# European-XFEL/xFrame

Hardware: AMD Instinct MI355X
Metric: MTIP iterations/sec, 128 q-shells x L_max=32 (higher is better)
Workload: dtype f64 (complex128); 1 GPU; BASELINE config 4: 128 shells x L_max=32, grid 128x64x128, 8 restarts per GPU on 3 streams, tutorial schedule (HIO/SW/ER, ft_stab on), fused step; restarts_per_gpu=8, restarts_total=8, streams_per_gpu=3, engines_take_turns=True, parallelism=restart-sharded x1, step_mode=fused

## Files before the change

### xframe_amd/csrc/k_sht.hip

```cpp
#include "mtip_internal.h"
#include "k_sht_common.h"
#include <cmath>
#include <cstdlib>

void build_legendre_tables(mtip_ctx* c, const double* cos_theta) {
    const int L = c->L, nt = c->nt;
    std::vector<int> poff(L + 2);
    for (int m = 0; m <= L + 1; ++m) poff[m] = m * (L + 1) - m * (m - 1) / 2;
    const size_t rows = (size_t)(L + 1) * (L + 2) / 2;
    std::vector<double> P(rows * nt);
    std::vector<double2> AB(rows, make_double2(0.0, 0.0));
    const double pi = 3.14159265358979323846;
    for (int t = 0; t < nt; ++t) {
        const double x = cos_theta[t];
        const double s = std::sqrt(std::fmax(0.0, 1.0 - x * x));
        double pmm = std::sqrt(1.0 / (4.0 * pi));
        for (int m = 0; m <= L; ++m) {
            if (m > 0) pmm = -std::sqrt((2.0 * m + 1.0) / (2.0 * m)) * s * pmm;
            P[(size_t)(poff[m]) * nt + t] = pmm;
            if (m < L) {
                double p2 = pmm;
                double p1 = std::sqrt(2.0 * m + 3.0) * x * pmm;
                P[(size_t)(poff[m] + 1) * nt + t] = p1;
                for (int l = m + 2; l <= L; ++l) {
                    const double a = std::sqrt((4.0 * l * l - 1.0) / ((double)l * l - (double)m * m));
                    const double b = std::sqrt((((double)l - 1.0) * (l - 1.0) - (double)m * m) / (4.0 * (l - 1.0) * (l - 1.0) - 1.0));
                    const double p = a * (x * p1 - b * p2);
                    P[(size_t)(poff[m] + l - m) * nt + t] = p;
                    AB[(size_t)poff[m] + l - m] = make_double2(a, b);
                    p2 = p1;
                    p1 = p;
                }
            }
        }
    }
    (void)mtip_copy(c, c->d_P, P.data(), P.size() * sizeof(double), hipMemcpyHostToDevice);
    (void)mtip_copy(c, c->d_poff, poff.data(), poff.size() * sizeof(int), hipMemcpyHostToDevice);
    if (c->d_AB != nullptr) (void)mtip_copy(c, c->d_AB, AB.data(), AB.size() * sizeof(double2), hipMemcpyHostToDevice);
    if (c->d_PT != nullptr) {
        const int nth = nt / 2;
        std::vector<double> PT((size_t)nth * rows);
        std::vector<int> lmtab(rows);
        for (int m = 0; m <= L; ++m)
            for (int l = m; l <= L; ++l) {
                const size_t idx = (size_t)poff[m] + l - m;
                lmtab[idx] = l | (m << 8);
                for (int t = 0; t < nth; ++t) PT[(size_t)t * rows + idx] = P[idx * nt + t];
            }
        (void)mtip_copy(c, c->d_PT, PT.data(), PT.size() * sizeof(double), hipMemcpyHostToDevice);
        (void)mtip_copy(c, c->d_lmtab, lmtab.data(), lmtab.size() * sizeof(int), hipMemcpyHostToDevice);
        c->chain_chunks = 0;
        if (c->d_PTc != nullptr) {
            std::vector<int> lmc(3 * 256, -1);
            std::vector<double> PTc((size_t)nth * 3 * 256, 0.0);
            int t = 0;
            bool fits = true;
            for (int m = 0; m <= L && fits; ++m)
                for (int par = 0; par < 2 && fits; ++par)
                    for (int l0 = m + par; l0 <= L; l0 += 6) {
                        if (t >= 256) { fits = false; break; }
                        for (int u = 0; u < 3; ++u) {
                            const int l = l0 + 2 * u;
// ... 191 lines not shown
            if (slot != nullptr) {
                const long long rows_per_b = (long long)Nq * nt;
                oo += (long long)slot[(row / rows_per_b) * SL_N + which] * B * rows_per_b * np;
            }
            if (EPI == EPI_MODULUS) {
                const double2 Fv = Fin[o];
                const double I = cabs2(Fv);
                const bool ok = (I >= 0.0) && (v.x >= 0.0);
                const double mult = ok ? sqrt(v.x / I) : 0.0;
                v = cscale(Fv, mult);
            } else if (EPI == EPI_SCALE_SHELL) {
                v = cscale(v, shell_scale[q]);
            }
            grid[oo] = v;
        }
    }
}

static void fft_launch_dims(const mtip_ctx* c, long long nrows, dim3* grid, dim3* block, size_t* smem) {
    const int T = c->np / 2;
    int R = 256 / T;
    if (R < 1) R = 1;
    *block = dim3((unsigned)(R * T));
    *grid = dim3((unsigned)div_up(nrows, R));
    *smem = (size_t)2 * R * c->np * sizeof(double2);
}

static constexpr size_t SHT_LDS_MAX = 160 * 1024, SHT_WIDE_LDS_MAX = 158 * 1024;

static size_t wide_lds(const mtip_ctx* c, int r1, int r2, int nsplit, int* rp) {
    if (c->nt % (2 * nsplit) != 0) return 0;
    const int ntl = c->nt / nsplit;
    if (nsplit > 1 && (ntl / 2) % 32 != 0) return 0;
    const size_t fixed = (nsplit > 1 ? 0 : (size_t)c->np) + (size_t)ntl * c->nm + c->npairs;
    auto bytes = [&](int v) { return (fixed + std::max((size_t)c->nlm, (size_t)v * r1 * (r2 + 1))) * sizeof(double2); };
    *rp = largest_even_divisor_le(ntl, std::min(SW_THREADS / r2, SW_THREADS / r1));
    while (*rp >= 2 && bytes(*rp) > SHT_WIDE_LDS_MAX) *rp = largest_even_divisor_le(ntl, *rp - 2);
    return *rp >= 2 ? bytes(*rp) : 0;
}

static void plan_chain(const mtip_ctx* c, int r1, int r2, ShtPlan& p) {
    if (c->np > 128) return;
    const int TP = c->nt / 2;
    for (int gsz = 64; gsz <= SW_THREADS; gsz *= 2) {
        const int maxi = div_up(c->npairs, gsz);
        if (TP % (SW_THREADS / gsz) != 0 || maxi > 3) continue;
        p.chain_gsz = gsz;
        p.chain_thg = TP / (SW_THREADS / gsz);
        const bool reg_tab = c->np == 128 && p.chain_thg == 16 && maxi >= 2;
        p.chain_maxi = reg_tab ? maxi : (maxi == 1 ? 1 : 3);
        p.chain = !reg_tab ? SHT_CHAIN_RT
                : (p.chain_maxi == 3 && c->L == 32 && c->nt == 64 && c->chain_chunks > 0) ? SHT_CHAIN_L32 : SHT_CHAIN_REGTAB;
        break;
    }
    if (p.chain == SHT_CHAIN_OFF) return;
    const size_t tb = (size_t)(SW_THREADS / 64) * (64 / r2) * r1 * (r2 + 1);
    const size_t fixed = (size_t)c->np + (size_t)c->nt * c->nm + c->npairs;
    p.chain_lds = (fixed + std::max(std::max((size_t)c->nlm, tb), (size_t)SW_THREADS * p.chain_maxi * 2)) * sizeof(double2);
    if (p.chain_lds > SHT_WIDE_LDS_MAX) p.chain = SHT_CHAIN_OFF;
}

void plan_sht(mtip_ctx* c) {
    int cap = 5;
    if (const char* e = std::getenv("MTIP_SHT_TIER")) cap = std::min(std::max(std::atoi(e), 0), 5);
    ShtPlan p;
    const int nt = c->nt, np = c->np;
    const size_t z = sizeof(double2);
    int r1 = 0, r2 = 0;
    if (cap >= 2 && nt % 2 == 0 && reg_radices(np, &r1, &r2)) {
        p.fwd_rp = largest_even_divisor_le(nt, std::min(2 * SR_THREADS / r2, SR_THREADS / r1));
        p.inv_rp = largest_even_divisor_le(nt, std::min(SR_THREADS / r2, SR_THREADS / r1));
        p.fwd_lds = ((size_t)np + (size_t)p.fwd_rp * r1 * (r2 + 1)) * z;
        p.inv_lds = ((size_t)np + c->nlm + (size_t)p.inv_rp * c->nm + (size_t)p.inv_rp * r1 * (r2 + 1)) * z;
        if (p.fwd_rp >= 2 && p.inv_rp >= 2 && p.fwd_lds <= SHT_LDS_MAX && p.inv_lds <= SHT_LDS_MAX) {
            p.fwd = SHT_FWD_REG;
            p.inv = SHT_INV_REG;
        }
    }
    if (p.fwd == SHT_FWD_REG) {
        const int per = div_up(c->npairs, SR_THREADS);
        p.fwd_maxi = per <= 3 ? 3 : per <= 5 ? 5 : 9;
        const int th = p.fwd_rp / 4;
        if (cap >= 3 && p.fwd_rp % 4 == 0 && (th == 2 || th == 4 || th == 8) && (nt / 2) % th == 0 && per <= 5) {
            p.fwd = SHT_FWD_PAIR;
            p.fwd_th = th;
            p.fwd_lds = ((size_t)np + (size_t)(p.fwd_rp / 2) * r1 * (r2 + 1)) * z;
        }
        for (int ns = 1; cap >= 3 && ns <= 2 && p.inv != SHT_INV_WIDE; ++ns) {
            int rp = 0;
            const size_t lds = wide_lds(c, r1, r2, ns, &rp);
            if (lds == 0) continue;
// ... 103 lines not shown
```

### xframe_amd/csrc/k_sht_chain.hip

```cpp
#include "mtip_internal.h"
#include "k_sht_common.h"
#include "k_sht_legendre.h"

#define CHAIN_STAMP(i)                           \
    if constexpr (DBG) stamp[i] = clock64();
#define CHAIN_SEG(i)                             \
    if constexpr (DBG) {                         \
        const long long n_ = clock64();          \
        stamp[i] += n_ - tprev;                  \
        tprev = n_;                              \
    }

struct ChainArgs {
    const double2* coeff;
    double2* grid;
    const double* P;
    const double2* AB;
    const double* cost;
    const double2* twN_g;
    const double2* Fin;
    const int* slot;
    const uint16_t* mk;
    RealEpi re;
    int npairs, nt, L, Nq, which, B;
    double2* coeff_out;
    const double* PT;
    const int* lmtab;
    const double* PTc;
    const int* lmc;
    const double* gw;
    double norm;
    long long* dbg;
    int gsz, thg;
};

template <int EPI, int PRE, int R1, int R2, int MAXI, int THG, bool DBG, int LC, bool CHK>
__global__ void __launch_bounds__(SW_THREADS) k_sht_chain(ChainArgs a) {
    constexpr int N = R1 * R2;
    constexpr int AS = R2 + 1;
    constexpr int GSR = R1 * AS;
    HIP_DYNAMIC_SHARED(double2, sm)
    long long stamp[DBG ? MTIP_CHAIN_DBG_SLOTS : 1];
    long long tprev = 0;
    if constexpr (DBG) {
#pragma unroll
        for (int i = 0; i < MTIP_CHAIN_DBG_SLOTS; ++i) stamp[i] = 0;
    }
    const int L = LC > 0 ? LC : a.L, nt = a.nt, npairs = LC > 0 ? (LC + 1) * (LC + 2) / 2 : a.npairs, Nq = a.Nq, B = a.B;
    const int nm = 2 * L + 1;
    const int nlm = (L + 1) * (L + 1);
    double2* twN = sm;
    double2* Gs = sm + N;
    double2* ABs = Gs + (size_t)nt * nm;
    double2* cl = ABs + npairs;
    double2* Bm = cl;
    const int tid = threadIdx.x;
    const long long shell = blockIdx.x;
    const int q = (int)(shell % Nq);
    const double2* csrc = a.coeff + (size_t)shell * nlm;
    const int wave = __builtin_amdgcn_readfirstlane(tid >> 6), nw = blockDim.x >> 6;
    CHAIN_STAMP(0)
    LegendreStart ls;
    legendre_prefetch_first(ls, a.P, nt, L, nt >> 1, 0, wave, tid & 63);
    for (int e = tid; e < N; e += blockDim.x) sm[e] = a.twN_g[e];
    for (int e = tid; e < npairs; e += blockDim.x) ABs[e] = a.AB[e];
    for (int e = tid; e < nlm; e += blockDim.x) cl[e] = csrc[e];
    long long dst_shell = shell;
    if (a.slot != nullptr && a.which >= 0) dst_shell += (long long)a.slot[(shell / Nq) * SL_N + a.which] * B * Nq;
    double2* gdst = a.grid + (size_t)dst_shell * nt * N;
    const double2* fsrc = a.Fin ? a.Fin + (size_t)shell * nt * N : nullptr;
    const double2* rprev = nullptr;
    const uint16_t* rmk = nullptr;
    double err_num = 0.0, err_den = 0.0;
    if (EPI == EPI_REAL_UPDATE) {
        const int bb = (int)(shell / Nq);
        const int* sl = a.slot + bb * SL_N;
        const size_t gsh = (size_t)nt * N;
        rprev = a.re.prev + ((size_t)sl[SL_CUR] * B * Nq + shell) * gsh;
        gdst = a.re.out + ((size_t)sl[SL_OUT] * B * Nq + shell) * gsh;
        rmk = a.mk + ((size_t)sl[SL_SUP] * B * Nq + shell) * nt * R2;
    }
    const int gsz = a.gsz;
    const int thg = THG > 0 ? THG : a.thg;
    const int grp = __builtin_amdgcn_readfirstlane(tid / gsz);
    const int tg = tid - grp * gsz;
    constexpr bool SPLIT = R2 == 16;
    constexpr int RW = 64 / R2;
    constexpr int S1 = RW * R1;
    static_assert(S1 * (SPLIT ? 2 : 1) <= 64, "lane roles");
    const int lane = tid & 63;
    const int n_grp = (nt + RW - 1) / RW;
    double2* Bw = Bm + (size_t)wave * (RW * R1 * AS);
    const int r2l = lane / R2, n2 = lane - r2l * R2;
    const int hf = SPLIT ? lane / S1 : 0;
    const int t1 = lane - hf * S1;
    const bool role1 = SPLIT || lane < S1;
    const int r1l = (t1 / R1) % RW, k1 = t1 % R1;
    constexpr bool HAS_PRE = EPI == EPI_MODULUS || EPI == EPI_REAL_UPDATE;
    double2 pre[HAS_PRE ? R1 : 1];
    unsigned pre_m = 0;
    double pre_w = 0.0;
    auto load_pre = [&](int g) {
        const int rr = g * RW + r2l;
        if (HAS_PRE && g < n_grp && rr < nt) {
            const int th = rr >> 1;
            const int row = (rr & 1) ? (nt - 1 - th) : th;
#pragma unroll
            for (int n1 = 0; n1 < R1; ++n1) {
                const size_t o = (size_t)row * N + R2 * n1 + n2;
                if (EPI == EPI_MODULUS) pre[n1] = fsrc[o];
                if (EPI == EPI_REAL_UPDATE) pre[n1] = rprev[o];
            }
            if (EPI == EPI_REAL_UPDATE) {
                pre_m = rmk[row * R2 + n2];
                pre_w = a.re.wt[row];
            }
        }
    };
    int my_lm[MAXI];
#pragma unroll
    for (int u = 0; u < MAXI; ++u) my_lm[u] = CHK ? a.lmc[u * 256 + tg] : a.lmtab[min(tg + u * gsz, npairs - 1)];
    __syncthreads();
    CHAIN_STAMP(1)
    load_pre(wave);
    const RealFlags rflags = real_flags(a.re.rp, a.re.method);
    const bool add_prev = EPI == EPI_REAL_UPDATE && a.re.add_prev && q > 0 && (a.re.add_mask == nullptr || a.re.add_mask[shell / Nq] != 0);
    const double wr_q = EPI == EPI_REAL_UPDATE ? a.re.wr[q] : 0.0;
    legendre_synthesis_rows(ls, Gs, cl, ABs, a.P, a.cost, nt, L, nt >> 1, 0, wave, nw, tid & 63);
    CHAIN_STAMP(2)
    __syncthreads();
    CHAIN_STAMP(3)
    if constexpr (DBG) tprev = stamp[3];
    for (int g = wave; g < n_grp; g += nw) {
        {
            const int rr = g * RW + r1l;
            if (role1 && rr < nt) {
                const double2* gr = Gs + (size_t)rr * nm + L;
                double2 uv[R2];
#pragma unroll
                for (int k2 = 0; k2 < R2; ++k2) {
                    const int k = k1 + R1 * k2;
                    const bool lo = k <= L, hi = k >= N - L;
                    const double2 v = gr[lo ? k : (hi ? k - N : 0)];
                    uv[k2] = (lo || hi) ? v : make_double2(0.0, 0.0);
                }
                double2* br = Bw + (size_t)(r1l * R1 + k1) * AS;
                if constexpr (SPLIT) {
                    double2 yv[R2 / 2];
                    half_fft<R2, true>(uv, hf, yv);
#pragma unroll
                    for (int j = 0; j < R2 / 2; ++j) {
                        const int m2 = 2 * j + hf;
                        double2 w = twN[m2 * k1];
                        w.y = -w.y;
                        br[m2] = cmul(yv[j], w);
                    }
                } else {
                    SmallFFT<R2, true>::run(uv);
#pragma unroll
                    for (int m2 = 0; m2 < R2; ++m2) {
                        double2 w = twN[m2 * k1];
// ... 14 lines not shown
            const double2* br = Bw + (size_t)r2l * R1 * AS + n2;
#pragma unroll
            for (int q1 = 0; q1 < R1; ++q1) vv[q1] = br[q1 * AS];
            SmallFFT<R1, true>::run(vv);
            const int th = rr2 >> 1;
            const int row = (rr2 & 1) ? (nt - 1 - th) : th;
#pragma unroll
            for (int n1 = 0; n1 < R1; ++n1) {
                double2 v = vv[n1];
                const size_t o = (size_t)row * N + R2 * n1 + n2;
                if (EPI == EPI_MODULUS) {
                    const double2 Fv = pre[n1];
                    const double I = cabs2(Fv);
                    const bool ok = (I >= 0.0) && (v.x >= 0.0);
                    const double mult = ok ? sqrt(v.x / I) : 0.0;
                    v = cscale(Fv, mult);
                } else if (EPI == EPI_REAL_UPDATE) {
                    const double2 pv = pre[n1];
                    const double2 w = add_prev ? cadd(v, pv) : v;
                    double2 Pj;
                    v = real_update_point_flat(a.re.rp, rflags, a.re.beta, w, pv, ((pre_m >> n1) & 1u) != 0, Pj);
                    if (!a.re.err_use_mask || ((pre_m >> (8 + n1)) & 1u)) {
                        const double wg = wr_q * pre_w;
                        const double dx = w.x - Pj.x, dy = w.y - Pj.y;
                        err_num = fma(wg, dx * dx + dy * dy, err_num);
                        err_den = fma(wg, w.x * w.x + w.y * w.y, err_den);
                    }
                }
                gdst[o] = v;
                if (PRE == MTIP_PRE_SQUARE) v = make_double2(cabs2(v), 0.0);
                vv[n1] = v;
            }
        }
        load_pre(g + nw);
#pragma unroll
        for (int n1 = 0; n1 < R1; ++n1) {
            const double px = __shfl_xor(vv[n1].x, R2, 64), py = __shfl_xor(vv[n1].y, R2, 64);
            vv[n1] = (r2l & 1) ? make_double2(px - vv[n1].x, py - vv[n1].y)
                               : make_double2(vv[n1].x + px, vv[n1].y + py);
        }
        if (act2) {
            SmallFFT<R1, false>::run(vv);
            double2* ar = Bw + (size_t)r2l * R1 * AS + n2;
#pragma unroll
            for (int q1 = 0; q1 < R1; ++q1) ar[q1 * AS] = cmul(vv[q1], twN[n2 * q1]);
        }
        MTIP_WAVE_LDS_SYNC();
        CHAIN_SEG(6)
        {
            const int rr = g * RW + r1l;
            if (role1 && rr < nt) {
                double2 uv[R2];
                const double2* ar = Bw + (size_t)(r1l * R1 + k1) * AS;
#pragma unroll
                for (int qq = 0; qq < R2; ++qq) uv[qq] = ar[qq];
                const double sc = a.gw[rr >> 1] * a.norm;
                double2* gr = Gs + (size_t)rr * nm + L;
                if constexpr (SPLIT) {
                    double2 yv[R2 / 2];
                    half_fft<R2, false>(uv, hf, yv);
#pragma unroll
                    for (int j = 0; j < R2 / 2; ++j) {
                        const int k = k1 + R1 * (2 * j + hf);
                        if (k <= L) gr[k] = cscale(yv[j], sc);
                        else if (k >= N - L) gr[k - N] = cscale(yv[j], sc);
                    }
                } else {
// ... 219 lines not shown
```

### xframe_amd/csrc/k_sht_legendre.h

```cpp
#pragma once
#include "mtip_internal.h"

struct LegendreStart {
    double pmm = 0.0, pm1 = 0.0;
};

__device__ __forceinline__ int legendre_item(int kk, int nw, int wave) { return kk * nw + ((kk & 1) ? nw - 1 - wave : wave); }

__device__ __forceinline__ void legendre_load_start(LegendreStart& s, const double* __restrict__ P, int nt, int L, int nth, int j0,
                                                    int n_chunks, int item, int lane) {
    const int jj = lane & 31, half_id = lane >> 5;
    const int mp = item / n_chunks, ch = item - mp * n_chunks;
    const int m = min(2 * mp + half_id, L);
    const int j = ch * 32 + jj;
    const int jc = j0 + (j < nth ? j : nth - 1);
    const double* pcol = P + (size_t)(m * (L + 1) - m * (m - 1) / 2) * nt + jc;
    s.pmm = pcol[0];
    s.pm1 = m < L ? pcol[nt] : 0.0;
}

__device__ __forceinline__ void legendre_prefetch_first(LegendreStart& s, const double* __restrict__ P, int nt, int L, int nth, int j0,
                                                        int wave, int lane) {
    const int n_chunks = (nth + 31) >> 5;
    const int n_items = ((L + 2) >> 1) * n_chunks;
    if (wave < n_items) legendre_load_start(s, P, nt, L, nth, j0, n_chunks, wave, lane);
}

__device__ __forceinline__ void legendre_synthesis_rows(LegendreStart& s, double2* __restrict__ Gs, const double2* __restrict__ cl,
                                                        const double2* __restrict__ ABs, const double* __restrict__ P,
                                                        const double* __restrict__ cost, int nt, int L, int nth, int j0,
                                                        int wave, int nw, int lane) {
    const int nm = 2 * L + 1;
    const int jj = lane & 31, half_id = lane >> 5;
    const int n_chunks = (nth + 31) >> 5;
    const int n_items = ((L + 2) >> 1) * n_chunks;
    for (int kk = 0;; ++kk) {
        const int i = legendre_item(kk, nw, wave);
        if (i >= n_items) break;
        const int mp = i / n_chunks, ch = i - mp * n_chunks;
        const int m_a = 2 * mp;
        const bool m_ok = m_a + half_id <= L;
        const int m = min(m_a + half_id, L);
        const int j = ch * 32 + jj;
        const bool act = (j < nth) && m_ok;
        const int jc = j0 + (j < nth ? j : nth - 1);
        const double x = cost[jc];
        double p2 = s.pmm, p1 = s.pm1;
        {
            const int i2 = legendre_item(kk + 1, nw, wave);
            if (i2 < n_items) legendre_load_start(s, P, nt, L, nth, j0, n_chunks, i2, lane);
        }
        const double2* cp = cl + m;
        const double2* cm = cl - m;
        const double2* abm = ABs + (m * (L + 1) - m * (m - 1) / 2) - m;
        double2 Ep, Em, Op = make_double2(0.0, 0.0), Om = make_double2(0.0, 0.0);
        {
            const double2 a = cp[m * (m + 1)], b = cm[m * (m + 1)];
            Ep = make_double2(p2 * a.x, p2 * a.y);
            Em = make_double2(p2 * b.x, p2 * b.y);
        }
        if (m < L) {
            const double2 a = cp[(m + 1) * (m + 2)], b = cm[(m + 1) * (m + 2)];
            Op = make_double2(p1 * a.x, p1 * a.y);
            Om = make_double2(p1 * b.x, p1 * b.y);
        }
        int l = m + 2;
        const int n_it = m_a + 2 <= L ? (L - m_a - 1) >> 1 : 0;
        double2 Aab0, Aab1, Acp, Aop, Acm, Aom, Bab0, Bab1, Bcp, Bop, Bcm, Bom;
#define LEG_LOAD(S, lq_)                                             \
        {                                                            \
            const int q_ = max(min((lq_), L - 1), 0);                \
            const int o_ = min((q_ + 1) * (q_ + 2), L * (L + 1));    \
            S##ab0 = abm[q_];                                        \
            S##ab1 = abm[q_ + 1];                                    \
            S##cp = cp[q_ * (q_ + 1)];                               \
            S##op = cp[o_];                                          \
            S##cm = cm[q_ * (q_ + 1)];                               \
            S##om = cm[o_];                                          \
        }
#define LEG_STEP(S)                                                         \
        if (l + 1 <= L) {                                                   \
            const double pa = S##ab0.x * (x * p1 - S##ab0.y * p2);          \
            const double pb = S##ab1.x * (x * pa - S##ab1.y * p1);          \
            Ep.x = fma(pa, S##cp.x, Ep.x); Ep.y = fma(pa, S##cp.y, Ep.y);   \
            Op.x = fma(pb, S##op.x, Op.x); Op.y = fma(pb, S##op.y, Op.y);   \
            Em.x = fma(pa, S##cm.x, Em.x); Em.y = fma(pa, S##cm.y, Em.y);   \
            Om.x = fma(pb, S##om.x, Om.x); Om.y = fma(pb, S##om.y, Om.y);   \
            p2 = pa;                                                        \
            p1 = pb;                                                        \
            l += 2;                                                         \
        }
#define LEG_PIN(S)                                                  \
        MTIP_PIN_VGPRS4(S##ab0.x, S##ab0.y, S##ab1.x, S##ab1.y)     \
        MTIP_PIN_VGPRS4(S##cp.x, S##cp.y, S##op.x, S##op.y)         \
        MTIP_PIN_VGPRS4(S##cm.x, S##cm.y, S##om.x, S##om.y)
        LEG_LOAD(A, l)
        for (int it = 0; it < n_it;) {
            LEG_LOAD(B, l + 2)
            LEG_STEP(A)
            LEG_PIN(B)
            if (++it >= n_it) break;
            LEG_LOAD(A, l + 2)
            LEG_STEP(B)
            LEG_PIN(A)
            ++it;
        }
#undef LEG_LOAD
#undef LEG_STEP
#undef LEG_PIN
        if (l <= L) {
            const double2 ab0 = abm[l];
            const double2 a = cp[l * (l + 1)], b = cm[l * (l + 1)];
            const double pa = ab0.x * (x * p1 - ab0.y * p2);
            Ep.x = fma(pa, a.x, Ep.x); Ep.y = fma(pa, a.y, Ep.y);
            Em.x = fma(pa, b.x, Em.x); Em.y = fma(pa, b.y, Em.y);
        }
        if (act) {
            double2* g_p = Gs + (size_t)(2 * j) * nm + L + m;
            g_p[0] = make_double2(Ep.x + Op.x, Ep.y + Op.y);
            g_p[nm] = make_double2(Ep.x - Op.x, Ep.y - Op.y);
            if (m > 0) {
                const double sg = (m & 1) ? -1.0 : 1.0;
                double2* g_m = Gs + (size_t)(2 * j) * nm + L - m;
                g_m[0] = make_double2(sg * (Em.x + Om.x), sg * (Em.y + Om.y));
                g_m[nm] = make_double2(sg * (Em.x - Om.x), sg * (Em.y - Om.y));
            }
        }
    }
}
```

### xframe_amd/csrc/k_sht_reg.hip

```cpp
#include "mtip_internal.h"
#include "k_sht_common.h"
#include "k_sht_legendre.h"

#define FWD_BATCH_MIN 5
template <int PRE, int R1, int R2, int MAXI>
__global__ void __launch_bounds__(SR_THREADS) k_sht_fwd_reg(const double2* __restrict__ grid, double2* __restrict__ coeff,
                                                            const double* __restrict__ PT, const int* __restrict__ lmtab,
                                                            const double2* __restrict__ twN_g, const double* __restrict__ gw,
                                                            int nt, int L, int npairs, int RP, double norm,
                                                            const int* __restrict__ slot, int which, int B, int Nq) {
    constexpr int N = R1 * R2;
    constexpr int AS = R2 + 1;
    HIP_DYNAMIC_SHARED(double2, sm)
    const int nm = 2 * L + 1;
    const int nlm = (L + 1) * (L + 1);
    double2* twN = sm;
    double2* A = twN + N;
    double2* G = A;
    const int tid = threadIdx.x;
    const long long shell = blockIdx.x;
    for (int e = tid; e < N; e += blockDim.x) twN[e] = twN_g[e];
    long long src_shell = shell;
    if (slot != nullptr) src_shell += (long long)slot[(shell / Nq) * SL_N + which] * B * Nq;
    const double2* gsrc = grid + (size_t)src_shell * nt * N;
// ... 369 lines not shown
                if (EPI == EPI_MODULUS) {
                    const double2 Fv = fsrc[o];
                    const double I = cabs2(Fv);
                    const bool ok = (I >= 0.0) && (v.x >= 0.0);
                    const double mult = ok ? sqrt(v.x / I) : 0.0;
                    v = cscale(Fv, mult);
                } else if (EPI == EPI_SCALE_SHELL) {
                    v = cscale(v, shell_scale[q]);
                }
                gdst[o] = v;
            }
        }
        __syncthreads();
    }
}

template <int EPI, int R1, int R2>
__global__ void __launch_bounds__(SW_THREADS) k_sht_inv_wide(const double2* __restrict__ coeff, double2* __restrict__ grid,
                                                             const double* __restrict__ P, const int* __restrict__ poff,
                                                             const double2* __restrict__ AB, const double* __restrict__ cost,
                                                             int npairs, const double2* __restrict__ twN_g, int nt, int L,
                                                             int RP, int Nq, const double2* __restrict__ Fin,
                                                             const double* __restrict__ shell_scale,
                                                             const int* __restrict__ slot, int which, int B,
                                                             const double2* __restrict__ coeff_sub, RealEpi re, int nsplit) {
    constexpr int N = R1 * R2;
    constexpr int AS = R2 + 1;
    HIP_DYNAMIC_SHARED(double2, sm)
    const int nm = 2 * L + 1;
    const int nlm = (L + 1) * (L + 1);
    const int ntl = nt / nsplit;
    const double2* twN = nsplit > 1 ? twN_g : sm;
    double2* Gs = sm + (nsplit > 1 ? 0 : N);
    double2* ABs = Gs + (size_t)ntl * nm;
    double2* cl = ABs + npairs;
    double2* Bm = cl;
    const int tid = threadIdx.x;
    const long long shell = blockIdx.x / nsplit;
    const int split = (int)(blockIdx.x - shell * nsplit);
    const int q = (int)(shell % Nq);
    const double2* csrc = coeff + (size_t)shell * nlm;
    const int wave = __builtin_amdgcn_readfirstlane(tid >> 6), nw = blockDim.x >> 6;
    const int nth = ntl >> 1;
    const int j0 = split * nth;
    LegendreStart ls;
    legendre_prefetch_first(ls, P, nt, L, nth, j0, wave, tid & 63);
    if (nsplit == 1)
        for (int e = tid; e < N; e += blockDim.x) sm[e] = twN_g[e];
    for (int e = tid; e < npairs; e += blockDim.x) ABs[e] = AB[e];
    if (coeff_sub != nullptr && q > 0) {
        const double2* ssrc = coeff_sub + (size_t)shell * nlm;
        for (int e = tid; e < nlm; e += blockDim.x) cl[e] = csub(csrc[e], ssrc[e]);
    } else {
        for (int e = tid; e < nlm; e += blockDim.x) cl[e] = csrc[e];
    }
    long long dst_shell = shell;
    if (slot != nullptr && which >= 0) dst_shell += (long long)slot[(shell / Nq) * SL_N + which] * B * Nq;
    double2* gdst = grid + (size_t)dst_shell * nt * N;
    const double2* fsrc = Fin ? Fin + (size_t)shell * nt * N : nullptr;
    const double2* rprev = nullptr;
    const uint8_t* rsup = nullptr;
    const uint8_t* rS0 = nullptr;
    double err_num = 0.0, err_den = 0.0;
    if (EPI == EPI_REAL_UPDATE) {
        const int bb = (int)(shell / Nq);
        const int* sl = slot + bb * SL_N;
        const size_t gsh = (size_t)nt * N;
        rprev = re.prev + ((size_t)sl[SL_CUR] * B * Nq + shell) * gsh;
        gdst = re.out + ((size_t)sl[SL_OUT] * B * Nq + shell) * gsh;
        rsup = re.sup + ((size_t)sl[SL_SUP] * B * Nq + shell) * gsh;
        rS0 = re.S0 + (size_t)q * gsh;
    }
    __syncthreads();
    legendre_synthesis_rows(ls, Gs, cl, ABs, P, cost, nt, L, nth, j0, wave, nw, tid & 63);
    __syncthreads();
    const int n_pass = ntl / RP;
    for (int pass = 0; pass < n_pass; ++pass) {
        double2 pre[(EPI == EPI_MODULUS || EPI == EPI_REAL_UPDATE) ? R1 : 1];
        uint8_t pre_s[EPI == EPI_REAL_UPDATE ? R1 : 1], pre_0[EPI == EPI_REAL_UPDATE ? R1 : 1];
        if ((EPI == EPI_MODULUS || EPI == EPI_REAL_UPDATE) && tid < RP * R2) {
            const int r = tid / R2, n2 = tid - r * R2;
            const int rr = pass * RP + r;
            const int th = j0 + (rr >> 1);
            const int row = (rr & 1) ? (nt - 1 - th) : th;
#pragma unroll
            for (int n1 = 0; n1 < R1; ++n1) {
                const size_t o = (size_t)row * N + R2 * n1 + n2;
                if (EPI == EPI_MODULUS) pre[n1] = fsrc[o];
                if (EPI == EPI_REAL_UPDATE) {
                    pre[n1] = rprev[o];
                    pre_s[n1] = rsup[o];
                    pre_0[n1] = re.err_use_mask ? rS0[o] : (uint8_t)1;
                }
            }
        }
        if (tid < RP * R1) {
            const int r = tid / R1, k1 = tid - r * R1;
            const double2* gr = Gs + (size_t)(pass * RP + r) * nm + L;
            double2 uv[R2];
#pragma unroll
            for (int k2 = 0; k2 < R2; ++k2) {
                const int k = k1 + R1 * k2;
                double2 v = make_double2(0.0, 0.0);
                if (k <= L) v = gr[k];
                else if (k >= N - L) v = gr[k - N];
                uv[k2] = v;
            }
// ... 158 lines not shown
```

### xframe_amd/csrc/mtip_api.hip

```cpp
#include "mtip_internal.h"
#include <algorithm>
#include <cmath>
#include <cstdlib>
#include <cstring>

static thread_local std::string g_create_error;

#define CTX_CHECK(c)                       \
    do {                                   \
        if ((c) == nullptr) return MTIP_EINVAL; \
    } while (0)
#define FAIL(c, code, msg)      \
    do {                        \
        (c)->err = (msg);       \
        return (code);          \
    } while (0)

static int post_launch(mtip_ctx* c, const char* what) {
    hipError_t e = hipGetLastError();
    if (e != hipSuccess) {
        c->err = std::string(what) + ": " + hipGetErrorString(e);
        return MTIP_EHIP;
    }
    return MTIP_OK;
// ... 68 lines not shown
    if (hipSetDevice(device) != hipSuccess) {
        g_create_error = "hipSetDevice failed";
        return nullptr;
    }
    mtip_ctx* c = new mtip_ctx();
    c->cfg = *cfg;
    c->device = device;
    c->N = cfg->n_radial;
    c->L = cfg->l_max;
    c->nt = cfg->n_theta;
    c->np = cfg->n_phi;
    c->B = cfg->n_batch;
    c->nlm = (c->L + 1) * (c->L + 1);
    c->nm = 2 * c->L + 1;
    c->Np = cfg->hankel_trapz ? c->N - 1 : c->N;
    c->G = (size_t)c->N * c->nt * c->np;
    c->C = (size_t)c->N * c->nlm;
    const int L = c->L, N = c->N, B = c->B;
    int rc = MTIP_OK;
    auto A = [&](int r) { if (rc == MTIP_OK) rc = r; };
    if (hipStreamCreateWithFlags(&c->stream, hipStreamNonBlocking) != hipSuccess) A(MTIP_EHIP);
    {
        int ncu = 0;
        if (hipDeviceGetAttribute(&ncu, hipDeviceAttributeMultiprocessorCount, device) == hipSuccess && ncu > 0) c->n_cu = ncu;
    }
    (void)hipEventCreate(&c->ev0);
    (void)hipEventCreate(&c->ev1);
    A(dev_alloc(c, &c->d_cost, c->nt));
    A(dev_alloc(c, &c->d_gw, c->nt));
    A(dev_alloc(c, &c->d_P, (size_t)(L + 1) * (L + 2) / 2 * c->nt));
    A(dev_alloc(c, &c->d_poff, L + 2));
    c->npairs = (L + 1) * (L + 2) / 2;
    A(dev_alloc(c, &c->d_PT, (size_t)(c->nt / 2 + 1) * c->npairs));
    A(dev_alloc(c, &c->d_AB, (size_t)c->npairs));
    A(dev_alloc(c, &c->d_lmtab, c->npairs));
    A(dev_alloc(c, &c->d_PTc, (size_t)(c->nt / 2 + 1) * 768));
    A(dev_alloc(c, &c->d_lmc, 768));
    if (const char* e = std::getenv("MTIP_DEG2_SIMPLE")) c->deg2_simple = std::atoi(e) != 0;
    if (const char* e = std::getenv("MTIP_HANKEL_CT")) {
        const int v = std::atoi(e);
        c->htile_force = (v == 1 || v == 2 || v == 3 || v == 5) ? v : 0;
    }
    if (rc == MTIP_OK) rc = build_hankel_tiles(c);
    A(dev_alloc(c, &c->d_twN, c->np));
    A(dev_alloc(c, &c->d_tw, c->np / 2));
    A(dev_alloc(c, &c->d_r, N));
    A(dev_alloc(c, &c->d_q, N));
    A(dev_alloc(c, &c->d_W, (size_t)(L + 1) * c->Np * N));
    c->kl.assign(L + 1, 0);
    c->used.assign(L + 1, 0);
    c->active.assign(L + 1, 0);
    c->voff.assign(L + 2, 0);
    c->xoff.assign(L + 2, 0);
    c->uoff.assign(L + 2, 0);
    c->have_V.assign(L + 1, 0);
    c->v_real.assign(L + 1, 1);
    c->psw = read_proj_switches();
    for (int l = 0; l <= L; ++l) {
        const int n = 2 * l + 1, k = std::min(n, N);
        c->kl[l] = k;
        c->voff[l + 1] = c->voff[l] + N * k;
        c->xoff[l + 1] = c->xoff[l] + k * n;
        c->uoff[l + 1] = c->uoff[l] + k * k;
    }
    c->vtot = c->voff[L + 1];
    c->xtot = c->xoff[L + 1];
    c->utot = c->uoff[L + 1];
// ... 1144 lines not shown
```

Baseline: 16260 MTIP iterations/s.

## Interleave Legendre recurrence coefficients with coefficients in LDS and deepen start-value prefetch

Rebuilds the LDS layout for Legendre synthesis into one interleaved record array per (m,l): the recurrence a/b factors sit beside the +m and -m spherical-harmonic coefficients, padded so each m has an extra entry. The inner loop can then fetch all operands for a step with contiguous loads, and the tail and bounds checks go away. The staging loop is batched with pinned registers and overlapped with lmtab/pre loads. Start values are prefetched through a multi-entry queue, and cos(theta) is cached in LDS or a register. This adds LDS footprint (three entries per record) and more register pressure.

```diff
diff --git a/xframe_amd/csrc/k_sht.hip b/xframe_amd/csrc/k_sht.hip
--- a/xframe_amd/csrc/k_sht.hip
+++ b/xframe_amd/csrc/k_sht.hip
@@ -1,5 +1,6 @@
 #include "mtip_internal.h"
 #include "k_sht_common.h"
+#include "k_sht_legendre.h"
 #include <cmath>
 #include <cstdlib>
 
@@ -9,7 +10,7 @@
     for (int m = 0; m <= L + 1; ++m) poff[m] = m * (L + 1) - m * (m - 1) / 2;
     const size_t rows = (size_t)(L + 1) * (L + 2) / 2;
     std::vector<double> P(rows * nt);
-    std::vector<double2> AB(rows, make_double2(0.0, 0.0));
+    std::vector<double2> AB((size_t)legendre_n_rec(L), make_double2(0.0, 0.0));
     const double pi = 3.14159265358979323846;
     for (int t = 0; t < nt; ++t) {
         const double x = cos_theta[t];
@@ -27,7 +28,7 @@
                     const double b = std::sqrt((((double)l - 1.0) * (l - 1.0) - (double)m * m) / (4.0 * (l - 1.0) * (l - 1.0) - 1.0));
                     const double p = a * (x * p1 - b * p2);
                     P[(size_t)(poff[m] + l - m) * nt + t] = p;
-                    AB[(size_t)poff[m] + l - m] = make_double2(a, b);
+                    AB[(size_t)legendre_rec(m, L) + l - m] = make_double2(a, b);
                     p2 = p1;
                     p1 = p;
                 }
@@ -285,8 +286,9 @@
     if (c->nt % (2 * nsplit) != 0) return 0;
     const int ntl = c->nt / nsplit;
     if (nsplit > 1 && (ntl / 2) % 32 != 0) return 0;
-    const size_t fixed = (nsplit > 1 ? 0 : (size_t)c->np) + (size_t)ntl * c->nm + c->npairs;
-    auto bytes = [&](int v) { return (fixed + std::max((size_t)c->nlm, (size_t)v * r1 * (r2 + 1))) * sizeof(double2); };
+    const size_t fixed = (nsplit > 1 ? 0 : (size_t)c->np) + (size_t)ntl * c->nm + (size_t)(ntl / 2 + 1) / 2;
+    const size_t recs = (size_t)legendre_lds_entries(c->L);
+    auto bytes = [&](int v) { return (fixed + std::max(recs, (size_t)v * r1 * (r2 + 1))) * sizeof(double2); };
     *rp = largest_even_divisor_le(ntl, std::min(SW_THREADS / r2, SW_THREADS / r1));
     while (*rp >= 2 && bytes(*rp) > SHT_WIDE_LDS_MAX) *rp = largest_even_divisor_le(ntl, *rp - 2);
     return *rp >= 2 ? bytes(*rp) : 0;
@@ -308,8 +310,8 @@
     }
     if (p.chain == SHT_CHAIN_OFF) return;
     const size_t tb = (size_t)(SW_THREADS / 64) * (64 / r2) * r1 * (r2 + 1);
-    const size_t fixed = (size_t)c->np + (size_t)c->nt * c->nm + c->npairs;
-    p.chain_lds = (fixed + std::max(std::max((size_t)c->nlm, tb), (size_t)SW_THREADS * p.chain_maxi * 2)) * sizeof(double2);
+    const size_t fixed = (size_t)c->np + (size_t)c->nt * c->nm + (size_t)(c->nt / 2 + 1) / 2;
+    p.chain_lds = (fixed + std::max(std::max((size_t)legendre_lds_entries(c->L), tb), (size_t)SW_THREADS * p.chain_maxi * 2)) * sizeof(double2);
     if (p.chain_lds > SHT_WIDE_LDS_MAX) p.chain = SHT_CHAIN_OFF;
 }
 
diff --git a/xframe_amd/csrc/k_sht_chain.hip b/xframe_amd/csrc/k_sht_chain.hip
--- a/xframe_amd/csrc/k_sht_chain.hip
+++ b/xframe_amd/csrc/k_sht_chain.hip
@@ -51,20 +51,22 @@
     const int nlm = (L + 1) * (L + 1);
     double2* twN = sm;
     double2* Gs = sm + N;
-    double2* ABs = Gs + (size_t)nt * nm;
-    double2* cl = ABs + npairs;
-    double2* Bm = cl;
+    double* cos_s = reinterpret_cast<double*>(Gs + (size_t)nt * nm);
+    double2* rec = Gs + (size_t)nt * nm + (nt / 2 + 1) / 2;
+    double2* Bm = rec;
     const int tid = threadIdx.x;
     const long long shell = blockIdx.x;
     const int q = (int)(shell % Nq);
     const double2* csrc = a.coeff + (size_t)shell * nlm;
     const int wave = __builtin_amdgcn_readfirstlane(tid >> 6), nw = blockDim.x >> 6;
     CHAIN_STAMP(0)
-    LegendreStart ls;
-    legendre_prefetch_first(ls, a.P, nt, L, nt >> 1, 0, wave, tid & 63);
-    for (int e = tid; e < N; e += blockDim.x) sm[e] = a.twN_g[e];
-    for (int e = tid; e < npairs; e += blockDim.x) ABs[e] = a.AB[e];
-    for (int e = tid; e < nlm; e += blockDim.x) cl[e] = csrc[e];
+    constexpr int LQ = 3;
+    constexpr bool L32 = LC == 32;
+    static_assert(!L32 || ((LC + 2) / 2 + SW_THREADS / 64 - 1) / (SW_THREADS / 64) <= LQ, "start-value queue");
+    unsigned add_m = 0;
+    if (EPI == EPI_REAL_UPDATE && a.re.add_mask != nullptr) add_m = a.re.add_mask[shell / Nq];
+    LegendreStart<LQ> ls;
+    legendre_prefetch<LQ, L32>(ls, a.P, a.cost, nt, L, nt >> 1, 0, wave, nw, tid & 63);
     long long dst_shell = shell;
     if (a.slot != nullptr && a.which >= 0) dst_shell += (long long)a.slot[(shell / Nq) * SL_N + a.which] * B * Nq;
     double2* gdst = a.grid + (size_t)dst_shell * nt * N;
@@ -100,9 +102,9 @@
     double2 pre[HAS_PRE ? R1 : 1];
     unsigned pre_m = 0;
     double pre_w = 0.0;
-    auto load_pre = [&](int g) {
-        const int rr = g * RW + r2l;
-        if (HAS_PRE && g < n_grp && rr < nt) {
+    auto load_pre = [&](int g, auto first) {
+        const int rr = first ? min(g * RW + r2l, nt - 1) : g * RW + r2l;
+        if (HAS_PRE && (first || (g < n_grp && rr < nt))) {
             const int th = rr >> 1;
             const int row = (rr & 1) ? (nt - 1 - th) : th;
 #pragma unroll
@@ -118,15 +120,21 @@
         }
     };
     int my_lm[MAXI];
-#pragma unroll
-    for (int u = 0; u < MAXI; ++u) my_lm[u] = CHK ? a.lmc[u * 256 + tg] : a.lmtab[min(tg + u * gsz, npairs - 1)];
+    const RealFlags rflags = real_flags(a.re.rp, a.re.method);
+    const double wr_q = EPI == EPI_REAL_UPDATE ? a.re.wr[q] : 0.0;
+    legendre_stage<false>(sm, a.twN_g, N, cos_s, a.cost, L32 ? 0 : nt >> 1, rec, a.AB, csrc, nullptr, L, tid, LC > 0 ? SW_THREADS : (int)blockDim.x, [&]() {
+#pragma unroll
+        for (int u = 0; u < MAXI; ++u) my_lm[u] = CHK ? a.lmc[u * 256 + tg] : a.lmtab[min(tg + u * gsz, npairs - 1)];
+        load_pre(wave, std::true_type());
+    });
+    if (EPI == EPI_REAL_UPDATE) {
+        unsigned z0 = 0, z1 = 0, z2 = 0;
+        MTIP_PIN_VGPRS4(add_m, z0, z1, z2)
+    }
+    const bool add_prev = EPI == EPI_REAL_UPDATE && a.re.add_prev && q > 0 && (a.re.add_mask == nullptr || add_m != 0);
     __syncthreads();
     CHAIN_STAMP(1)
-    load_pre(wave);
-    const RealFlags rflags = real_flags(a.re.rp, a.re.method);
-    const bool add_prev = EPI == EPI_REAL_UPDATE && a.re.add_prev && q > 0 && (a.re.add_mask == nullptr || a.re.add_mask[shell / Nq] != 0);
-    const double wr_q = EPI == EPI_REAL_UPDATE ? a.re.wr[q] : 0.0;
-    legendre_synthesis_rows(ls, Gs, cl, ABs, a.P, a.cost, nt, L, nt >> 1, 0, wave, nw, tid & 63);
+    legendre_synthesis_rows<LQ, !L32, L32>(ls, Gs, rec, cos_s, a.P, nt, L, nt >> 1, 0, wave, nw, tid & 63);
     CHAIN_STAMP(2)
     __syncthreads();
     CHAIN_STAMP(3)
@@ -207,7 +215,7 @@
                 vv[n1] = v;
             }
         }
-        load_pre(g + nw);
+        load_pre(g + nw, std::false_type());
 #pragma unroll
         for (int n1 = 0; n1 < R1; ++n1) {
             const double px = __shfl_xor(vv[n1].x, R2, 64), py = __shfl_xor(vv[n1].y, R2, 64);
diff --git a/xframe_amd/csrc/k_sht_legendre.h b/xframe_amd/csrc/k_sht_legendre.h
--- a/xframe_amd/csrc/k_sht_legendre.h
+++ b/xframe_amd/csrc/k_sht_legendre.h
@@ -1,85 +1,154 @@
 #pragma once
 #include "mtip_internal.h"
 
+constexpr int LEG_AHEAD = 12;
+
+__host__ __device__ inline int legendre_rec(int m, int L) { return m * (L + 2) - m * (m - 1) / 2; }
+__host__ __device__ inline int legendre_n_rec(int L) { return (L + 1) * (L + 2) / 2 + L + 1; }
+__host__ __device__ inline int legendre_lds_entries(int L) { return 3 * legendre_n_rec(L) + LEG_AHEAD; }
+
+template <int NQ>
 struct LegendreStart {
-    double pmm = 0.0, pm1 = 0.0;
+    double pmm[NQ], pm1[NQ];
+    double x = 0.0;
 };
 
 __device__ __forceinline__ int legendre_item(int kk, int nw, int wave) { return kk * nw + ((kk & 1) ? nw - 1 - wave : wave); }
 
-__device__ __forceinline__ void legendre_load_start(LegendreStart& s, const double* __restrict__ P, int nt, int L, int nth, int j0,
-                                                    int n_chunks, int item, int lane) {
+__device__ __forceinline__ void legendre_load_start(double& pmm, double& pm1, const double* __restrict__ P, int nt, int L, int nth,
+                                                    int j0, int n_chunks, int item, int lane) {
     const int jj = lane & 31, half_id = lane >> 5;
-    const int mp = item / n_chunks, ch = item - mp * n_chunks;
+    const int mp = n_chunks == 1 ? item : item / n_chunks, ch = item - mp * n_chunks;
     const int m = min(2 * mp + half_id, L);
     const int j = ch * 32 + jj;
     const int jc = j0 + (j < nth ? j : nth - 1);
     const double* pcol = P + (size_t)(m * (L + 1) - m * (m - 1) / 2) * nt + jc;
-    s.pmm = pcol[0];
-    s.pm1 = m < L ? pcol[nt] : 0.0;
-}
-
-__device__ __forceinline__ void legendre_prefetch_first(LegendreStart& s, const double* __restrict__ P, int nt, int L, int nth, int j0,
-                                                        int wave, int lane) {
-    const int n_chunks = (nth + 31) >> 5;
+    pmm = pcol[0];
+    const double v = pcol[m < L ? nt : 0];
+    pm1 = m < L ? v : 0.0;
+}
+
+template <int NQ, bool ONECH>
+__device__ __forceinline__ void legendre_prefetch(LegendreStart<NQ>& s, const double* __restrict__ P, const double* __restrict__ cost,
+                                                  int nt, int L, int nth, int j0, int wave, int nw, int lane) {
+    const int n_chunks = ONECH ? 1 : (nth + 31) >> 5;
     const int n_items = ((L + 2) >> 1) * n_chunks;
-    if (wave < n_items) legendre_load_start(s, P, nt, L, nth, j0, n_chunks, wave, lane);
-}
-
-__device__ __forceinline__ void legendre_synthesis_rows(LegendreStart& s, double2* __restrict__ Gs, const double2* __restrict__ cl,
-                                                        const double2* __restrict__ ABs, const double* __restrict__ P,
-                                                        const double* __restrict__ cost, int nt, int L, int nth, int j0,
-                                                        int wave, int nw, int lane) {
+#pragma unroll
+    for (int u = 0; u < NQ; ++u)
+        legendre_load_start(s.pmm[u], s.pm1[u], P, nt, L, nth, j0, n_chunks, min(legendre_item(u, nw, wave), n_items - 1), lane);
+    if (ONECH) s.x = cost[j0 + min(lane & 31, nth - 1)];
+}
+
+template <bool SUB, class Younger>
+__device__ __forceinline__ void legendre_stage(double2* __restrict__ tw_s, const double2* __restrict__ tw_g, int n_tw,
+                                               double* __restrict__ cos_s, const double* __restrict__ cost, int n_cos,
+                                               double2* __restrict__ rec, const double2* __restrict__ ABp,
+                                               const double2* __restrict__ csrc, const double2* __restrict__ ssrc, int L, int tid, int nthr,
+                                               Younger&& younger) {
+    constexpr int NA = 2, NC = 4;
+    const int n_rec = legendre_n_rec(L), nlm = (L + 1) * (L + 1), n_co = (L + 2) * (L + 2);
+    const int n_ch = max(max((n_tw + nthr - 1) / nthr, (n_cos + nthr - 1) / nthr),
+                         max((n_rec + NA * nthr - 1) / (NA * nthr), (n_co + NC * nthr - 1) / (NC * nthr)));
+    for (int c = 0; c < n_ch; ++c) {
+        const int e1 = c * nthr + tid;
+        double2 vt = tw_g[max(min(e1, n_tw - 1), 0)];
+        double vx = cost[max(min(e1, n_cos - 1), 0)];
+        double2 va[NA], vc[NC], vs[SUB ? NC : 1];
+#pragma unroll
+        for (int u = 0; u < NA; ++u) va[u] = ABp[min((c * NA + u) * nthr + tid, n_rec - 1)];
+#pragma unroll
+        for (int u = 0; u < NC; ++u) {
+            const int e = min((c * NC + u) * nthr + tid, nlm - 1);
+            vc[u] = csrc[e];
+            if (SUB) vs[u] = ssrc[e];
+        }
+        asm volatile("" ::: "memory");
+        if (c == 0) younger();
+        double pz = 0.0;
+        MTIP_PIN_VGPRS4(vt.x, vt.y, vx, pz)
+#pragma unroll
+        for (int u = 0; u < NA; u += 2) { MTIP_PIN_VGPRS4(va[u].x, va[u].y, va[u + 1].x, va[u + 1].y) }
+#pragma unroll
+        for (int u = 0; u < NC; u += 2) { MTIP_PIN_VGPRS4(vc[u].x, vc[u].y, vc[u + 1].x, vc[u + 1].y) }
+        if (SUB) {
+#pragma unroll
+            for (int u = 0; u < NC; u += 2) { MTIP_PIN_VGPRS4(vs[u].x, vs[u].y, vs[SUB ? u + 1 : 0].x, vs[SUB ? u + 1 : 0].y) }
+        }
+        if (e1 < n_tw) tw_s[e1] = vt;
+        if (e1 < n_cos) cos_s[e1] = vx;
+#pragma unroll
+        for (int u = 0; u < NA; ++u) {
+            const int e = (c * NA + u) * nthr + tid;
+            if (e < n_rec) rec[3 * e] = va[u];
+        }
+#pragma unroll
+        for (int u = 0; u < NC; ++u) {
+            const int e = (c * NC + u) * nthr + tid;
+            const int l = (int)sqrtf((float)e + 0.5f);
+            const int mq = e - l * (l + 1), ma = mq < 0 ? -mq : mq;
+            if (e < n_co && ma <= L) {
+                double2 v = SUB ? csub(vc[u], vs[u]) : vc[u];
+                if (e >= nlm) v = make_double2(0.0, 0.0);
+                double2* r = rec + 3 * (legendre_rec(ma, L) + l - ma);
+                if (mq >= 0) r[1] = v;
+                if (mq <= 0) r[2] = v;
+            }
+        }
+    }
+}
+
+template <int NQ, bool REFILL, bool ONECH>
+__device__ __forceinline__ void legendre_synthesis_rows(LegendreStart<NQ>& s, double2* __restrict__ Gs, const double2* __restrict__ rec,
+                                                        const double* __restrict__ cos_s, const double* __restrict__ P,
+                                                        int nt, int L, int nth, int j0, int wave, int nw, int lane) {
     const int nm = 2 * L + 1;
     const int jj = lane & 31, half_id = lane >> 5;
-    const int n_chunks = (nth + 31) >> 5;
+    const int n_chunks = ONECH ? 1 : (nth + 31) >> 5;
     const int n_items = ((L + 2) >> 1) * n_chunks;
     for (int kk = 0;; ++kk) {
         const int i = legendre_item(kk, nw, wave);
         if (i >= n_items) break;
-        const int mp = i / n_chunks, ch = i - mp * n_chunks;
+        const int mp = ONECH ? i : i / n_chunks, ch = i - mp * n_chunks;
         const int m_a = 2 * mp;
         const bool m_ok = m_a + half_id <= L;
         const int m = min(m_a + half_id, L);
         const int j = ch * 32 + jj;
         const bool act = (j < nth) && m_ok;
-        const int jc = j0 + (j < nth ? j : nth - 1);
-        const double x = cost[jc];
-        double p2 = s.pmm, p1 = s.pm1;
+        const double x = ONECH ? s.x : cos_s[j < nth ? j : nth - 1];
+        double p2 = s.pmm[0], p1 = s.pm1[0];
+#pragma unroll
+        for (int u = 0; u + 1 < NQ; ++u) {
+            s.pmm[u] = s.pmm[u + 1];
+            s.pm1[u] = s.pm1[u + 1];
+        }
+        if (REFILL) {
+            const int i2 = legendre_item(kk + NQ, nw, wave);
+            if (i2 < n_items) legendre_load_start(s.pmm[NQ - 1], s.pm1[NQ - 1], P, nt, L, nth, j0, n_chunks, i2, lane);
+        }
+        const double2* r = rec + 3 * legendre_rec(m, L);
+        double2 Ep, Em, Op, Om;
         {
-            const int i2 = legendre_item(kk + 1, nw, wave);
-            if (i2 < n_items) legendre_load_start(s, P, nt, L, nth, j0, n_chunks, i2, lane);
-        }
-        const double2* cp = cl + m;
-        const double2* cm = cl - m;
-        const double2* abm = ABs + (m * (L + 1) - m * (m - 1) / 2) - m;
-        double2 Ep, Em, Op = make_double2(0.0, 0.0), Om = make_double2(0.0, 0.0);
-        {
-            const double2 a = cp[m * (m + 1)], b = cm[m * (m + 1)];
+            const double2 a = r[1], b = r[2], c = r[4], d = r[5];
             Ep = make_double2(p2 * a.x, p2 * a.y);
             Em = make_double2(p2 * b.x, p2 * b.y);
-        }
-        if (m < L) {
-            const double2 a = cp[(m + 1) * (m + 2)], b = cm[(m + 1) * (m + 2)];
-            Op = make_double2(p1 * a.x, p1 * a.y);
-            Om = make_double2(p1 * b.x, p1 * b.y);
-        }
-        int l = m + 2;
+            Op = make_double2(p1 * c.x, p1 * c.y);
+            Om = make_double2(p1 * d.x, p1 * d.y);
+        }
+        r += 6;
         const int n_it = m_a + 2 <= L ? (L - m_a - 1) >> 1 : 0;
+        const bool tail = m_a + 2 <= L && ((L - m_a) & 1) == 0;
         double2 Aab0, Aab1, Acp, Aop, Acm, Aom, Bab0, Bab1, Bcp, Bop, Bcm, Bom;
-#define LEG_LOAD(S, lq_)                                             \
+#define LEG_LOAD(S, q_)                                              \
         {                                                            \
-            const int q_ = max(min((lq_), L - 1), 0);                \
-            const int o_ = min((q_ + 1) * (q_ + 2), L * (L + 1));    \
-            S##ab0 = abm[q_];                                        \
-            S##ab1 = abm[q_ + 1];                                    \
-            S##cp = cp[q_ * (q_ + 1)];                               \
-            S##op = cp[o_];                                          \
-            S##cm = cm[q_ * (q_ + 1)];                               \
-            S##om = cm[o_];                                          \
+            S##ab0 = (q_)[0];                                        \
+            S##cp = (q_)[1];                                         \
+            S##cm = (q_)[2];                                         \
+            S##ab1 = (q_)[3];                                        \
+            S##op = (q_)[4];                                         \
+            S##om = (q_)[5];                                         \
         }
 #define LEG_STEP(S)                                                         \
-        if (l + 1 <= L) {                                                   \
+        {                                                                   \
             const double pa = S##ab0.x * (x * p1 - S##ab0.y * p2);          \
             const double pb = S##ab1.x * (x * pa - S##ab1.y * p1);          \
             Ep.x = fma(pa, S##cp.x, Ep.x); Ep.y = fma(pa, S##cp.y, Ep.y);   \
@@ -88,32 +157,42 @@
             Om.x = fma(pb, S##om.x, Om.x); Om.y = fma(pb, S##om.y, Om.y);   \
             p2 = pa;                                                        \
             p1 = pb;                                                        \
-            l += 2;                                                         \
         }
 #define LEG_PIN(S)                                                  \
         MTIP_PIN_VGPRS4(S##ab0.x, S##ab0.y, S##ab1.x, S##ab1.y)     \
         MTIP_PIN_VGPRS4(S##cp.x, S##cp.y, S##op.x, S##op.y)         \
-        MTIP_PIN_VGPRS4(S##cm.x, S##cm.y, S##om.x, S##om.y)
-        LEG_LOAD(A, l)
-        for (int it = 0; it < n_it;) {
-            LEG_LOAD(B, l + 2)
+        MTIP_PIN_VGPRS4(S##cm.x, S##cm.y, S##om.x, S##om.y)         \
+        asm volatile("" ::: "memory");
+        LEG_LOAD(A, r)
+        LEG_LOAD(B, r + 6)
+        int it = n_it;
+        if (it >= 2) {
+            do {
+                LEG_PIN(A)
+                LEG_STEP(A)
+                LEG_LOAD(A, r + 12)
+                LEG_PIN(B)
+                LEG_STEP(B)
+                LEG_LOAD(B, r + 18)
+                r += 12;
+                it -= 2;
+            } while (it >= 2);
+        }
+        LEG_PIN(A)
+        if (it) {
             LEG_STEP(A)
             LEG_PIN(B)
-            if (++it >= n_it) break;
-            LEG_LOAD(A, l + 2)
-            LEG_STEP(B)
-            LEG_PIN(A)
-            ++it;
+            Aab0 = Bab0;
+            Acp = Bcp;
+            Acm = Bcm;
         }
 #undef LEG_LOAD
 #undef LEG_STEP
 #undef LEG_PIN
-        if (l <= L) {
-            const double2 ab0 = abm[l];
-            const double2 a = cp[l * (l + 1)], b = cm[l * (l + 1)];
-            const double pa = ab0.x * (x * p1 - ab0.y * p2);
-            Ep.x = fma(pa, a.x, Ep.x); Ep.y = fma(pa, a.y, Ep.y);
-            Em.x = fma(pa, b.x, Em.x); Em.y = fma(pa, b.y, Em.y);
+        if (tail) {
+            const double pa = Aab0.x * (x * p1 - Aab0.y * p2);
+            Ep.x = fma(pa, Acp.x, Ep.x); Ep.y = fma(pa, Acp.y, Ep.y);
+            Em.x = fma(pa, Acm.x, Em.x); Em.y = fma(pa, Acm.y, Em.y);
         }
         if (act) {
             double2* g_p = Gs + (size_t)(2 * j) * nm + L + m;
diff --git a/xframe_amd/csrc/k_sht_reg.hip b/xframe_amd/csrc/k_sht_reg.hip
--- a/xframe_amd/csrc/k_sht_reg.hip
+++ b/xframe_amd/csrc/k_sht_reg.hip
@@ -425,9 +425,9 @@
     const int ntl = nt / nsplit;
     const double2* twN = nsplit > 1 ? twN_g : sm;
     double2* Gs = sm + (nsplit > 1 ? 0 : N);
-    double2* ABs = Gs + (size_t)ntl * nm;
-    double2* cl = ABs + npairs;
-    double2* Bm = cl;
+    double* cos_s = reinterpret_cast<double*>(Gs + (size_t)ntl * nm);
+    double2* rec = Gs + (size_t)ntl * nm + (ntl / 2 + 1) / 2;
+    double2* Bm = rec;
     const int tid = threadIdx.x;
     const long long shell = blockIdx.x / nsplit;
     const int split = (int)(blockIdx.x - shell * nsplit);
@@ -436,17 +436,13 @@
     const int wave = __builtin_amdgcn_readfirstlane(tid >> 6), nw = blockDim.x >> 6;
     const int nth = ntl >> 1;
     const int j0 = split * nth;
-    LegendreStart ls;
-    legendre_prefetch_first(ls, P, nt, L, nth, j0, wave, tid & 63);
-    if (nsplit == 1)
-        for (int e = tid; e < N; e += blockDim.x) sm[e] = twN_g[e];
-    for (int e = tid; e < npairs; e += blockDim.x) ABs[e] = AB[e];
-    if (coeff_sub != nullptr && q > 0) {
-        const double2* ssrc = coeff_sub + (size_t)shell * nlm;
-        for (int e = tid; e < nlm; e += blockDim.x) cl[e] = csub(csrc[e], ssrc[e]);
-    } else {
-        for (int e = tid; e < nlm; e += blockDim.x) cl[e] = csrc[e];
-    }
+    constexpr int NQ = 4;
+    LegendreStart<NQ> ls;
+    legendre_prefetch<NQ, false>(ls, P, cost, nt, L, nth, j0, wave, nw, tid & 63);
+    if (coeff_sub != nullptr && q > 0)
+        legendre_stage<true>(sm, twN_g, nsplit == 1 ? N : 0, cos_s, cost + j0, nth, rec, AB, csrc, coeff_sub + (size_t)shell * nlm, L, tid, (int)blockDim.x, []() {});
+    else
+        legendre_stage<false>(sm, twN_g, nsplit == 1 ? N : 0, cos_s, cost + j0, nth, rec, AB, csrc, nullptr, L, tid, (int)blockDim.x, []() {});
     long long dst_shell = shell;
     if (slot != nullptr && which >= 0) dst_shell += (long long)slot[(shell / Nq) * SL_N + which] * B * Nq;
     double2* gdst = grid + (size_t)dst_shell * nt * N;
@@ -465,7 +461,7 @@
         rS0 = re.S0 + (size_t)q * gsh;
     }
     __syncthreads();
-    legendre_synthesis_rows(ls, Gs, cl, ABs, P, cost, nt, L, nth, j0, wave, nw, tid & 63);
+    legendre_synthesis_rows<NQ, true, false>(ls, Gs, rec, cos_s, P, nt, L, nth, j0, wave, nw, tid & 63);
     __syncthreads();
     const int n_pass = ntl / RP;
     for (int pass = 0; pass < n_pass; ++pass) {
diff --git a/xframe_amd/csrc/mtip_api.hip b/xframe_amd/csrc/mtip_api.hip
--- a/xframe_amd/csrc/mtip_api.hip
+++ b/xframe_amd/csrc/mtip_api.hip
@@ -124,7 +124,7 @@
     A(dev_alloc(c, &c->d_poff, L + 2));
     c->npairs = (L + 1) * (L + 2) / 2;
     A(dev_alloc(c, &c->d_PT, (size_t)(c->nt / 2 + 1) * c->npairs));
-    A(dev_alloc(c, &c->d_AB, (size_t)c->npairs));
+    A(dev_alloc(c, &c->d_AB, (size_t)c->npairs + L + 1));
     A(dev_alloc(c, &c->d_lmtab, c->npairs));
     A(dev_alloc(c, &c->d_PTc, (size_t)(c->nt / 2 + 1) * 768));
     A(dev_alloc(c, &c->d_lmc, 768));
```

Measured after the change: 17140 MTIP iterations/s, median of 6. 5.4% higher.
